# dominikh/jello

Hardware: AMD Instinct MI355X
Metric: Mpixels/sec fine-raster + paths/sec, 100k-path 4096^2 scene (higher is better)
Workload: dtype f32

## Files before the change

### jello_amd/csrc/kernels_coarse.hip

```cpp
#include <cstring>

#include "kcommon.h"

using namespace jk;
using namespace jd;

namespace {

struct Cmd {
    const JlConfig* cfg;
    JlBump* bump;
    Buf<uint32_t> ptcl;
    uint32_t cmd_offset, cmd_limit;
    uint32_t dyn_start;
    uint32_t chunk_base;
    uint32_t chunk_words;
    uint32_t seg_base, seg_used;
};

struct __attribute__((packed, aligned(4))) PtclQuad { uint32_t a, b, c, d; };
JD void ptcl_wr4(const Buf<uint32_t>& ptcl, uint32_t i, uint32_t a, uint32_t b, uint32_t c, uint32_t d) {
    if (i + 3u < ptcl.n && i + 3u >= i) {
        PtclQuad q; q.a = a; q.b = b; q.c = c; q.d = d;
        *(PtclQuad*)(ptcl.p + i) = q;
    } else {
        ptcl.wr(i, a); ptcl.wr(i + 1u, b); ptcl.wr(i + 2u, c); ptcl.wr(i + 3u, d);
    }
}

#ifndef COARSE_POOL_CHUNKS
#define COARSE_POOL_CHUNKS 16u
#endif
template <int MODE>
JD void alloc_cmd(Cmd& c, uint32_t size) {
    const bool need = c.cmd_offset + size >= c.cmd_limit;
    uint32_t new_cmd = c.dyn_start + c.chunk_base + c.chunk_words;
    if (MODE == 1) {
        if (need) {
            if (new_cmd + JL_PTCL_INCREMENT > c.cfg->ptcl_size) {
                new_cmd = 0u;
                atomicOr(&c.bump->failed, (uint32_t)JL_STAGE_COARSE);
            }
            c.ptcl.wr(c.cmd_offset, JL_CMD_JUMP);
            c.ptcl.wr(c.cmd_offset + 1u, new_cmd);
        }
    }
    c.chunk_words += need ? JL_PTCL_INCREMENT : 0u;
    c.cmd_offset = need ? new_cmd : c.cmd_offset;
    c.cmd_limit = need ? new_cmd + (JL_PTCL_INCREMENT - JL_PTCL_HEADROOM) : c.cmd_limit;
}

#define COARSE_UNROLL 4u
#ifndef COARSE_TILE_CACHE
#define COARSE_TILE_CACHE 1536u
#endif
#ifndef COARSE_WG_PER_CU
#define COARSE_WG_PER_CU 2u
#endif
#ifndef COARSE_MAX_SPLIT
#define COARSE_MAX_SPLIT 16u
#endif
#ifndef COARSE_PAR_WG_PER_CU
#define COARSE_PAR_WG_PER_CU 4u
#endif

#define CM_CLIP 1u
#define CM_BLEND 2u
#define CM_EVENODD_INCLUDE 4u
#define CM_EVENODD_FILL 8u
#define CM_PATH 16u
#define CM_BEGIN 32u
#define CM_END 64u
#define CM_NBRUSH_SHIFT 8u

#ifndef COARSE_TPL
#define COARSE_TPL 1u
#endif
#if COARSE_TPL != 1
#error "the write pass derives a tile's bases from its thread index: one tile per lane"
#endif
struct Walk {
    Cmd c;
    uint32_t blend_offset, clip_zero_depth, clip_depth, render_blend_depth, max_blend_depth;
    uint32_t tile_x, tile_y, my_xy, slot;
    bool has_tile;
    uint32_t slice_ix, bitmap, nz, el_next;
    uint4 q0, q2;
    JlTile tile;
};

struct CoarseReloc {
    uint32_t* arena_ctr;
    uint2* owner;
    unsigned long long* masks;
    uint32_t* aux;
    uint32_t* end_pos;
};

template <int MODE, bool CLIPS>
__global__ __launch_bounds__(JL_WG) void k_coarse(const JlConfig* __restrict__ cfg, Buf<uint32_t> scene, Buf<JlDrawMonoid> draw_monoids,
                                                  Buf<JlBinHeader> bin_headers, Buf<uint32_t> info_bin_data, Buf<JlPath> paths, Buf<JlTile> tiles,
                                                  JlBump* __restrict__ bump, Buf<uint32_t> ptcl, uint32_t* __restrict__ cnt_seg,
                                                  uint32_t* __restrict__ cnt_chunk, uint32_t* __restrict__ cnt_blend,
                                                  uint32_t* __restrict__ wg_tot, uint32_t n_wg, uint32_t bin_row0, uint32_t split, CoarseReloc R) {
    constexpr bool WRITE = MODE != 0;
    const uint32_t bin_y = blockIdx.y + bin_row0;
    const uint32_t part_rows = JL_N_TILE_Y / split, part_y0 = blockIdx.z * part_rows, part_y1 = part_y0 + part_rows;
    __shared__ uint32_t sh_bitmaps[8][JL_N_TILE];
    __shared__ uint32_t sh_part_count[JL_WG];
    __shared__ uint32_t sh_part_offsets[JL_WG];
    __shared__ uint32_t sh_drawobj_ix[JL_WG];
    __shared__ uint32_t sh_tile_count[JL_WG];
    __shared__ uint4 sh_r0[JL_WG];
    __shared__ uint4 sh_r1[JL_WG];
    __shared__ uint4 sh_r2[JL_WG];
    __shared__ uint32_t sh_scan[8];
    __shared__ uint32_t sh_red[12];
    constexpr bool PAR = MODE == 2;
    __shared__ uint2 sh_tile_cache[PAR ? 1u : COARSE_TILE_CACHE];
    __shared__ uint32_t sh_st[8][PAR ? JL_N_TILE : 1u];
    __shared__ uint8_t sh_list[JL_WG / 64][2][PAR ? JL_N_TILE : 1u];
    __shared__ uint32_t sh_pool[JL_WG / 64][2];
    if (PAR && threadIdx.x < JL_WG / 64) { sh_pool[threadIdx.x][0] = 0u; sh_pool[threadIdx.x][1] = 0u; }

    const uint32_t lid = threadIdx.x;
    const uint32_t width_in_bins = (cfg->width_in_tiles + JL_N_TILE_X - 1u) / JL_N_TILE_X;
    const uint32_t bin_ix = width_in_bins * bin_y + blockIdx.x;
    if (bin_ix * split + blockIdx.z >= n_wg) return;
    const uint32_t part_tiles = part_rows * JL_N_TILE_X, walkers = part_tiles / COARSE_TPL;
    Walk W[COARSE_TPL];
#pragma unroll
    for (uint32_t k = 0; k < COARSE_TPL; k++) {
        W[k].has_tile = lid < walkers;
        const uint32_t t = W[k].has_tile ? lid + k * walkers : 0u;
        W[k].tile_x = t % JL_N_TILE_X;
        W[k].tile_y = part_y0 + t / JL_N_TILE_X;
        W[k].my_xy = W[k].tile_y * JL_N_TILE_X + W[k].tile_x;
        W[k].slot = bin_ix * JL_N_TILE + W[k].my_xy;
    }

    {
        uint32_t failed = bump->failed & (JL_STAGE_BINNING | JL_STAGE_TILE_ALLOC | JL_STAGE_FLATTEN);
        if (bump->seg_counts > cfg->seg_counts_size) failed |= JL_STAGE_PATH_COUNT;
        if (failed != 0u) {
            if (WRITE) {
                if (blockIdx.x == 0u && blockIdx.y == 0u && lid == 0u) atomicOr(&bump->failed, failed);
            }
            if (MODE != 1) {
#pragma unroll
                for (uint32_t k = 0; k < COARSE_TPL; k++)
                    if (W[k].has_tile) { cnt_seg[W[k].slot] = 0u; cnt_chunk[W[k].slot] = 0u; cnt_blend[W[k].slot] = 0u; }
                if (lid < 3u) wg_tot[lid * n_wg + bin_ix * split + blockIdx.z] = 0u;
            }
            if (MODE == 2) {
#pragma unroll
                for (uint32_t k = 0; k < COARSE_TPL; k++)
                    if (W[k].has_tile) R.end_pos[W[k].slot] = 0xffffffffu;
            }
            return;
        }
    }
    const uint32_t n_partitions = (cfg->layout.n_drawobj + JL_N_TILE - 1u) / JL_N_TILE;
    const uint32_t bin_tile_x = JL_N_TILE_X * blockIdx.x;
    const uint32_t bin_tile_y = JL_N_TILE_Y * bin_y;
    const uint32_t BLEND_CLIP = (128u << 8) | 0u;
    uint32_t my_base_seg = 0u, my_base_chunk = 0u, my_base_blend = 0u;
    if (MODE == 1) {
        const uint32_t my_wg = bin_ix * split + blockIdx.z;
        MonoidK<3> before, all;
#pragma unroll
        for (int c = 0; c < 3; c++) { before.v[c] = 0u; all.v[c] = 0u; }
        const bool totals = blockIdx.x == 0u && blockIdx.y == 0u && blockIdx.z == 0u;
        for (uint32_t j = lid; j < (totals ? n_wg : my_wg); j += JL_WG) {
#pragma unroll
            for (int c = 0; c < 3; c++) {
                const uint32_t v = wg_tot[(uint32_t)c * n_wg + j];
                all.v[c] += v;
                if (j < my_wg) before.v[c] += v;
            }
        }
        const MonoidK<3> carry = block_reduce_monoid<3>(before, sh_red);
        __syncthreads();
        if (totals) {
            const MonoidK<3> t = block_reduce_monoid<3>(all, sh_red);
            if (lid == 0u) { bump->segments = t.v[0]; bump->ptcl = t.v[1]; bump->blend = t.v[2]; }
            __syncthreads();
        }
        const bool mine = W[0].has_tile;
        uint32_t tot;
        my_base_seg = carry.v[0] + block_excl_scan_u32(mine ? cnt_seg[W[0].slot] : 0u, sh_scan, &tot);
        __syncthreads();
        my_base_chunk = carry.v[1] + block_excl_scan_u32(mine ? cnt_chunk[W[0].slot] : 0u, sh_scan, &tot);
        __syncthreads();
        my_base_blend = carry.v[2] + block_excl_scan_u32(mine ? cnt_blend[W[0].slot] : 0u, sh_scan, &tot);
        __syncthreads();
    }
#pragma unroll
    for (uint32_t k = 0; k < COARSE_TPL; k++) {
        Walk& w = W[k];
        const uint32_t this_tile_ix = (bin_tile_y + w.tile_y) * cfg->width_in_tiles + bin_tile_x + w.tile_x;
        w.c.cfg = cfg; w.c.bump = bump; w.c.ptcl = ptcl;
        w.c.cmd_offset = this_tile_ix * JL_PTCL_INITIAL_ALLOC;
        w.c.cmd_limit = w.c.cmd_offset + (JL_PTCL_INITIAL_ALLOC - JL_PTCL_HEADROOM);
        w.c.dyn_start = cfg->width_in_tiles * cfg->height_in_tiles * JL_PTCL_INITIAL_ALLOC;
        w.c.chunk_base = my_base_chunk;
        w.c.chunk_words = 0u;
        w.c.seg_base = my_base_seg;
        w.c.seg_used = 0u;
        if (MODE == 2 && w.has_tile && bin_tile_x + w.tile_x < cfg->width_in_tiles && bin_tile_y + w.tile_y < cfg->height_in_tiles &&
            (size_t)this_tile_ix * JL_PTCL_INITIAL_ALLOC + JL_PTCL_INITIAL_ALLOC <= ptcl.n) {
            R.masks[(size_t)this_tile_ix * 2u] = 0ull;
            R.masks[(size_t)this_tile_ix * 2u + 1u] = 0ull;
        }
        w.clip_zero_depth = 0u; w.clip_depth = 0u; w.render_blend_depth = 0u; w.max_blend_depth = 0u;
        w.blend_offset = w.c.cmd_offset;
        w.c.cmd_offset += 1u;
        w.slice_ix = 7u; w.bitmap = 0u; w.nz = 0u; w.el_next = 0xffffffffu;
        w.q0 = make_uint4(0u, 0u, 0u, 0u); w.q2 = w.q0;
        w.tile.backdrop = 0; w.tile.segment_count_or_ix = 0u;
    }
    if constexpr (PAR) {
        if (W[0].has_tile) {
            sh_st[0][lid] = W[0].c.cmd_offset; sh_st[1][lid] = W[0].c.cmd_limit; sh_st[2][lid] = 0u; sh_st[3][lid] = 0u;
            sh_st[4][lid] = 0u; sh_st[5][lid] = 0u; sh_st[6][lid] = 0u; sh_st[7][lid] = 0u;
        }
    }
    uint32_t partition_ix = 0u, rd_ix = 0u, wr_ix = 0u, part_start_ix = 0u, ready_ix = 0u;

    auto gather = [&]() -> uint32_t {
        for (;;) {
            if (ready_ix == wr_ix && partition_ix < n_partitions) {
                part_start_ix = ready_ix;
                uint32_t count = 0u;
                if (partition_ix + lid < n_partitions) {
                    uint32_t in_ix = (partition_ix + lid) * JL_N_TILE + bin_ix;
                    JlBinHeader bh = bin_headers.rd(in_ix);
                    count = bh.element_count;
                    sh_part_offsets[lid] = bh.chunk_offset;
                }
                uint32_t tot;
                uint32_t excl = block_excl_scan_u32(count, sh_scan, &tot);
                sh_part_count[lid] = part_start_ix + excl + count;
                __syncthreads();
                ready_ix = sh_part_count[JL_WG - 1u];
                partition_ix += JL_WG;
            }
            uint32_t ix = rd_ix + lid;
            if (ix >= wr_ix && ix < ready_ix) {
                uint32_t part_ix = 0u;
                for (uint32_t i = 0; i < 8u; i++) {
                    uint32_t probe = part_ix + (128u >> i);
                    if (ix >= sh_part_count[probe - 1u]) part_ix = probe;
                }
                ix -= (part_ix > 0u) ? sh_part_count[part_ix - 1u] : part_start_ix;
                uint32_t offset = cfg->layout.bin_data_start + sh_part_offsets[part_ix];
                sh_drawobj_ix[lid] = info_bin_data.rd(offset + ix);
            }
            wr_ix = umin_(rd_ix + JL_N_TILE, ready_ix);
            if (wr_ix - rd_ix >= JL_N_TILE || (wr_ix >= ready_ix && partition_ix >= n_partitions)) break;
            __syncthreads();
        }
        return (lid + rd_ix < wr_ix) ? sh_drawobj_ix[lid] : 0xffffffffu;
    };
    uint32_t n_tag = JL_DRAWTAG_NOP;
    JlDrawMonoid n_dm;
    n_dm.path_ix = 0u; n_dm.clip_ix = 0u; n_dm.scene_offset = 0u; n_dm.info_offset = 0u;
    auto stage1 = [&](uint32_t obj) {
        n_tag = JL_DRAWTAG_NOP;
        if (obj != 0xffffffffu) {
            n_tag = scene.rd(cfg->layout.drawtag_base + obj);
            n_dm = draw_monoids.rd(obj);
        }
    };
    uint4 n_r0 = make_uint4(0u, 0u, 0u, 0u), n_r1 = make_uint4(0u, 0u, 0u, 0u), n_r2 = make_uint4(0u, 0u, 0u, 0u);
    uint32_t n_tile_count = 0u;
    auto stage2 = [&]() {
        const uint32_t tag = n_tag;
        n_tile_count = 0u;
        n_r0 = make_uint4(0u, 0u, 0u, 0u); n_r1 = make_uint4(0u, 0u, 0u, 0u); n_r2 = make_uint4(0u, 0u, 0u, 0u);
        if (tag != JL_DRAWTAG_NOP) {
            const JlDrawMonoid dm0 = n_dm;
            uint32_t path_ix = dm0.path_ix;
            uint32_t dd0 = cfg->layout.drawdata_base + dm0.scene_offset;
            const uint32_t di = dm0.info_offset;
            const uint32_t draw_flags = info_bin_data.rd(di);
            const uint4 sc = make_uint4(scene.rd(dd0), scene.rd(dd0 + 1u), scene.rd(dd0 + 2u), scene.rd(dd0 + 3u));
            uint32_t meta = (draw_flags & 1u) != 0u ? CM_EVENODD_INCLUDE : 0u;
            if ((tag & 1u) != 0u) {
                meta |= CM_CLIP;
                if (sc.x != BLEND_CLIP) meta |= CM_BLEND;
            }
            if (tag == JL_DRAWTAG_FILL_COLOR) {
                meta |= CM_PATH | (meta & CM_EVENODD_INCLUDE ? CM_EVENODD_FILL : 0u) | (5u << CM_NBRUSH_SHIFT);
                n_r0.y = JL_CMD_COLOR; n_r2 = sc;
            } else if (tag == JL_DRAWTAG_FILL_LIN_GRADIENT || tag == JL_DRAWTAG_FILL_RAD_GRADIENT || tag == JL_DRAWTAG_FILL_SWEEP_GRADIENT) {
                meta |= CM_PATH | (meta & CM_EVENODD_INCLUDE ? CM_EVENODD_FILL : 0u) | (3u << CM_NBRUSH_SHIFT);
                n_r0.y = tag == JL_DRAWTAG_FILL_LIN_GRADIENT ? JL_CMD_LIN_GRAD : (tag == JL_DRAWTAG_FILL_RAD_GRADIENT ? JL_CMD_RAD_GRAD : JL_CMD_SWEEP_GRAD);
                n_r2.x = sc.x; n_r2.y = di + 1u;
            } else if (tag == JL_DRAWTAG_FILL_IMAGE) {
                meta |= CM_PATH | (meta & CM_EVENODD_INCLUDE ? CM_EVENODD_FILL : 0u) | (2u << CM_NBRUSH_SHIFT);
                n_r0.y = JL_CMD_IMAGE; n_r2.x = di + 1u;
            } else if (CLIPS && tag == JL_DRAWTAG_BEGIN_CLIP) {
                meta |= CM_BEGIN | (1u << CM_NBRUSH_SHIFT);
                n_r0.y = JL_CMD_BEGIN_CLIP;
            } else if (CLIPS && tag == JL_DRAWTAG_END_CLIP) {
                meta |= CM_END | CM_PATH | (3u << CM_NBRUSH_SHIFT);
                n_r0.y = JL_CMD_END_CLIP; n_r2.x = sc.x; n_r2.y = sc.y;
            }
            n_r0.x = meta;
            JlPath path = paths.rd(path_ix);
            uint32_t stride = path.bbox[2] - path.bbox[0];
            n_r0.w = stride;
            int32_t dx = (int32_t)path.bbox[0] - (int32_t)bin_tile_x;
            int32_t dy = (int32_t)path.bbox[1] - (int32_t)bin_tile_y;
            int32_t x0 = iclamp_(dx, 0, JL_N_TILE_X);
            int32_t y0 = iclamp_(dy, (int32_t)part_y0, (int32_t)part_y1);
            int32_t x1 = iclamp_((int32_t)path.bbox[2] - (int32_t)bin_tile_x, 0, JL_N_TILE_X);
            int32_t y1 = iclamp_((int32_t)path.bbox[3] - (int32_t)bin_tile_y, (int32_t)part_y0, (int32_t)part_y1);
            {
                const uint32_t wdt = (uint32_t)(x1 - x0);
                n_r1.y = wdt | ((wdt ? (65536u + wdt - 1u) / wdt : 0u) << 5);
            }
            n_r1.x = (uint32_t)x0 | ((uint32_t)y0 << 16);
            n_tile_count = (uint32_t)(x1 - x0) * (uint32_t)(y1 - y0);
            n_r0.z = path.tiles - (uint32_t)(dy * (int32_t)stride + dx);
        }
    };
    stage1(gather());
    stage2();
    for (;;) {
        for (uint32_t i = 0; i < 8u; i++) sh_bitmaps[i][lid] = 0u;
        const uint32_t tile_count = n_tile_count;
        uint4 r0 = n_r0, r1 = n_r1, r2 = n_r2;
        uint32_t total_tile_count;
        uint32_t excl_tc = block_excl_scan_u32(tile_count, sh_scan, &total_tile_count);
        sh_tile_count[lid] = excl_tc + tile_count;
        r1.z = excl_tc;
        sh_r0[lid] = r0; sh_r1[lid] = r1; sh_r2[lid] = r2;
        __syncthreads();
        rd_ix += JL_N_TILE;
        const bool has_next = !(rd_ix >= ready_ix && partition_ix >= n_partitions);
        if (has_next) stage1(gather());
        uint32_t win_e0 = 0u, win_p0 = 0u;
        bool did_stage2 = false;
        for (;;) {
        uint32_t win_e1 = PAR ? JL_N_TILE : win_e0;
        for (uint32_t step = 256u; step > 0u && !PAR; step >>= 1)
            if (win_e1 + step <= JL_N_TILE && sh_tile_count[win_e1 + step - 1u] - win_p0 <= COARSE_TILE_CACHE) win_e1 += step;
        const uint32_t win_p1 = sh_tile_count[win_e1 - 1u];
        for (uint32_t base = win_p0; base < win_p1; base += COARSE_UNROLL * JL_N_TILE) {
            uint32_t p_el[COARSE_UNROLL], p_xy[COARSE_UNROLL], p_tile[COARSE_UNROLL];
            JlTile p_t[COARSE_UNROLL];
#pragma unroll
            for (uint32_t u = 0; u < COARSE_UNROLL; u++) {
                const uint32_t ix = base + u * JL_N_TILE + lid;
                p_el[u] = 0xffffffffu; p_xy[u] = 0u; p_tile[u] = 0u;
                p_t[u].backdrop = 0; p_t[u].segment_count_or_ix = 0u;
                if (ix < win_p1) {
                    uint32_t el_ix = 0u;
#pragma unroll
                    for (uint32_t i = 0; i < 8u; i++) {
                        uint32_t probe = el_ix + (128u >> i);
                        if (ix >= sh_tile_count[probe - 1u]) el_ix = probe;
                    }
                    const uint4 q0 = sh_r0[el_ix], q1 = sh_r1[el_ix];
                    uint32_t seq_ix = ix - q1.z;
                    uint32_t width = q1.y & 31u;
                    uint32_t row = (seq_ix * (q1.y >> 5)) >> 16;
                    uint32_t x = (q1.x & 0xffffu) + (seq_ix - row * width);
                    uint32_t y = (q1.x >> 16) + row;
                    p_el[u] = el_ix;
                    p_xy[u] = y * JL_N_TILE_X + x;
                    p_tile[u] = q0.z + q0.w * y + x;
                }
            }
#pragma unroll
            for (uint32_t u = 0; u < COARSE_UNROLL; u++)
                if (p_el[u] != 0xffffffffu) p_t[u] = tiles.rd(p_tile[u]);
#pragma unroll
            for (uint32_t u = 0; u < COARSE_UNROLL; u++) {
                if (p_el[u] == 0xffffffffu) continue;
                const uint32_t ix = base + u * JL_N_TILE + lid;
                const uint32_t el_ix = p_el[u];
                const JlTile tile = p_t[u];
                if (!PAR) sh_tile_cache[ix - win_p0] = make_uint2((uint32_t)tile.backdrop, tile.segment_count_or_ix);
                const uint32_t meta = sh_r0[el_ix].x;
                const bool is_clip = (meta & CM_CLIP) != 0u, is_blend = (meta & CM_BLEND) != 0u;
                const bool even_odd = (meta & CM_EVENODD_INCLUDE) != 0u;
                uint32_t n_segs = tile.segment_count_or_ix;
                int32_t bd = tile.backdrop;
                int32_t absbd = bd < 0 ? (int32_t)(0u - (uint32_t)bd) : bd;
                bool backdrop_clear = (even_odd ? (absbd & 1) : bd) == 0;
                bool include_tile = n_segs != 0u || (backdrop_clear == is_clip) || is_blend;
                if (include_tile) atomicOr(&sh_bitmaps[el_ix / 32u][p_xy[u]], 1u << (el_ix & 31u));
            }
        }
        if (has_next && !did_stage2) { stage2(); did_stage2 = true; }
        __syncthreads();
        if constexpr (PAR) {
            const uint32_t wv = lid >> 6, lane = lid & 63u;
            const uint64_t below = (1ull << lane) - 1ull, above = ~below & ~(1ull << lane);
            auto mbcnt64 = [&](uint64_t m) -> uint32_t { return __builtin_amdgcn_mbcnt_hi((uint32_t)(m >> 32), __builtin_amdgcn_mbcnt_lo((uint32_t)m, 0u)); };
            auto prepare = [&](uint32_t t, uint32_t buf, uint32_t& e_out, JlTile& tl) -> uint32_t {
                e_out = 0u; tl.backdrop = 0; tl.segment_count_or_ix = 0u;
                if (t >= part_tiles) return 0u;
                const uint32_t ty = part_y0 + t / JL_N_TILE_X, tx = t % JL_N_TILE_X, xy = ty * JL_N_TILE_X + tx;
                uint32_t n = 0u;
#pragma unroll
                for (uint32_t c = 0u; c < 4u; c++) {
                    const uint64_t m = (uint64_t)uni(sh_bitmaps[2u * c][xy]) | ((uint64_t)uni(sh_bitmaps[2u * c + 1u][xy]) << 32);
                    if (m != 0ull) {
                        if ((m >> lane) & 1ull) sh_list[wv][buf][(n + mbcnt64(m)) & 255u] = (uint8_t)(64u * c + lane);
                        n += (uint32_t)__builtin_popcountll(m);
                    }
                }
                wave_sync();
                if (lane < n) {
                    e_out = sh_list[wv][buf][lane];
                    const uint4 q0 = sh_r0[e_out];
                    tl = tiles.rd(q0.z + q0.w * ty + tx);
                }
                return n;
            };
            uint32_t nx_e; JlTile nx_tile;
            uint32_t nx_n = prepare(wv, 0u, nx_e, nx_tile);
            uint32_t buf = 0u;
            for (uint32_t t = wv; t < part_tiles; t += JL_WG / 64u, buf ^= 1u) {
                const uint32_t n = nx_n, e_first = nx_e;
                const JlTile tile_first = nx_tile;
                nx_n = prepare(t + JL_WG / 64u, buf ^ 1u, nx_e, nx_tile);
                if (n == 0u) continue;
                const uint32_t ty = part_y0 + t / JL_N_TILE_X, tx = t % JL_N_TILE_X;
                const uint32_t slot = bin_ix * JL_N_TILE + ty * JL_N_TILE_X + tx;
                uint32_t off = uni(sh_st[0][t]), lim = uni(sh_st[1][t]), chunkw = uni(sh_st[2][t]), segused = uni(sh_st[3][t]);
                uint32_t czd = uni(sh_st[4][t]), depth = uni(sh_st[5][t]), rbd = uni(sh_st[6][t]), maxbd = uni(sh_st[7][t]);
                const uint32_t dyn_start = cfg->width_in_tiles * cfg->height_in_tiles * JL_PTCL_INITIAL_ALLOC;
                for (uint32_t k0 = 0u; k0 < n; k0 += 64u) {
                    const bool live = k0 + lane < n;
                    uint32_t e = e_first;
                    JlTile tile = tile_first;
                    if (k0 != 0u) {
                        e = live ? sh_list[wv][buf][k0 + lane] : 0u;
                        tile.backdrop = 0; tile.segment_count_or_ix = 0u;
                        if (live) { const uint4 t0 = sh_r0[e]; tile = tiles.rd(t0.z + t0.w * ty + tx); }
                    }
                    const uint4 q0 = sh_r0[e], q2 = sh_r2[e];
                    const uint32_t meta = live ? q0.x : 0u;
                    const uint32_t n_segs = live ? tile.segment_count_or_ix : 0u;
                    const uint32_t is_begin = (meta / CM_BEGIN) & 1u, is_end = (meta / CM_END) & 1u, has_path = (meta / CM_PATH) & 1u;
                    const uint32_t has_segs = umin_(n_segs, 1u);
                    const uint32_t zero_tile = live ? 1u - umin_(n_segs | (uint32_t)tile.backdrop, 1u) : 0u;
                    const uint32_t dlt = is_begin - is_end;
                    const uint32_t d_incl = wave_incl_scan_u32(dlt);
                    const uint32_t D = depth + d_incl - dlt;
                    const uint64_t begins = __builtin_amdgcn_ballot_w64(is_begin != 0u);
                    const uint64_t zb = __builtin_amdgcn_ballot_w64((is_begin & zero_tile) != 0u);
                    uint32_t has_partner = 0u, partner_empty = 0u, matched = 0u;
                    for (uint64_t todo = begins; todo != 0ull;) {
                        const uint32_t L = (uint32_t)__builtin_amdgcn_readlane((int)D, (int)__builtin_ctzll(todo));
                        const bool bl_me = is_begin != 0u && D == L, el_me = is_end != 0u && D == L + 1u;
                        const uint64_t bl = __builtin_amdgcn_ballot_w64(bl_me), el = __builtin_amdgcn_ballot_w64(el_me);
                        if (el_me) {
                            const uint64_t c = bl & below;
                            if (c != 0ull) { has_partner = 1u; partner_empty = (uint32_t)(zb >> (63u - (uint32_t)__builtin_clzll(c))) & 1u; }
                        }
                        if (bl_me) {
                            const uint64_t ea = el & above, ba = bl & above;
                            matched = (ea != 0ull && (ba == 0ull || __builtin_ctzll(ea) < __builtin_ctzll(ba))) ? 1u : 0u;
                        }
                        todo &= ~bl;
                    }
                    const uint64_t ze = __builtin_amdgcn_ballot_w64((is_end & partner_empty) != 0u);
                    uint32_t skipped = mbcnt64(zb) > mbcnt64(ze) ? 1u : 0u;
                    uint32_t czd_out;
                    bool entered_persists = false;
                    if (czd != 0u) {
                        const uint64_t fin = __builtin_amdgcn_ballot_w64(is_end != 0u && has_partner == 0u && D == czd);
                        const uint32_t endl = fin != 0ull ? (uint32_t)__builtin_ctzll(fin) : 64u;
                        if (lane <= endl) skipped = 1u;
                        entered_persists = fin == 0ull;
                    }
                    if (entered_persists) {
                        czd_out = czd;
                    } else {
                        const uint64_t open_z = __builtin_amdgcn_ballot_w64((is_begin & zero_tile) != 0u && matched == 0u);
                        czd_out = open_z != 0ull ? (uint32_t)__builtin_amdgcn_readlane((int)D, (int)__builtin_ctzll(open_z)) + 1u : 0u;
                    }
                    const uint32_t active = 1u - skipped;
                    const uint32_t opened = is_begin & active & (1u - zero_tile), closes = is_end & active;
                    const uint32_t rd = opened - closes;
                    const uint32_t r_incl = wave_incl_scan_u32(rd);
                    const uint32_t peak = rbd + r_incl - rd + opened;
                    maxbd = umax_(maxbd, (uint32_t)__builtin_amdgcn_readlane((int)wave_incl_max_u32(peak), 63));
                    rbd += (uint32_t)__builtin_amdgcn_readlane((int)r_incl, 63);
                    depth += (uint32_t)__builtin_amdgcn_readlane((int)d_incl, 63);
                    czd = czd_out;
                    const uint32_t emit_path = active & has_path;
                    const uint32_t emit_brush = active & (1u - (is_begin & zero_tile));
                    const uint32_t s1 = emit_path * (1u + 3u * has_segs);
                    const uint32_t s2 = emit_brush * ((meta >> CM_NBRUSH_SHIFT) & 7u);
                    const uint32_t segs_here = emit_path * n_segs;
                    const uint32_t sg_incl = wave_incl_scan_u32(segs_here);
                    const uint32_t seg_ix = segused + sg_incl - segs_here;
                    segused += (uint32_t)__builtin_amdgcn_readlane((int)sg_incl, 63);
                    const uint32_t sz_incl = wave_incl_scan_u32(s1 + s2);
                    uint32_t o1 = off + sz_incl - (s1 + s2), o2 = o1 + s1;
                    uint32_t fl = 0u, fslot = 0u;
                    for (uint32_t guard = 0u; guard < 130u; guard++) {
                        const bool at1 = lane > fl || (lane == fl && fslot == 0u), at2 = lane >= fl;
                        const uint64_t m1 = __builtin_amdgcn_ballot_w64(s1 != 0u && at1 && o1 + s1 >= lim);
                        const uint64_t m2 = __builtin_amdgcn_ballot_w64(s2 != 0u && at2 && o2 + s2 >= lim);
                        if ((m1 | m2) == 0ull) break;
                        const uint32_t l1 = m1 != 0ull ? (uint32_t)__builtin_ctzll(m1) : 64u, l2 = m2 != 0ull ? (uint32_t)__builtin_ctzll(m2) : 64u;
                        const uint32_t bl = l1 <= l2 ? l1 : l2, bslot = l1 <= l2 ? 0u : 1u;
                        const uint32_t bo = (uint32_t)__builtin_amdgcn_readlane((int)(bslot == 0u ? o1 : o2), (int)bl);
                        uint32_t pn = uni(sh_pool[wv][0]), pe = uni(sh_pool[wv][1]);
                        if (pe - pn < JL_PTCL_INCREMENT) {
                            const uint32_t grab = COARSE_POOL_CHUNKS * JL_PTCL_INCREMENT;
                            uint32_t base = 0u;
                            if (lane == 0u) base = atomicAdd(R.arena_ctr, grab);
                            base = uni(base);
                            if (lane >= 1u && lane < COARSE_POOL_CHUNKS && dyn_start + base + lane * JL_PTCL_INCREMENT + JL_PTCL_INCREMENT <= ptcl.n)
                                R.owner[base / JL_PTCL_INCREMENT + lane] = make_uint2(0xffffffffu, 0u);
                            pn = base; pe = base + grab;
                        }
                        wave_sync();
                        if (lane == 0u) { sh_pool[wv][0] = pn + JL_PTCL_INCREMENT; sh_pool[wv][1] = pe; }
                        wave_sync();
                        uint32_t new_cmd = dyn_start + pn;
                        if (new_cmd + JL_PTCL_INCREMENT > ptcl.n || new_cmd + JL_PTCL_INCREMENT < new_cmd) {
                            new_cmd = 0u;
                        } else {
                            if (lane == 0u) R.owner[pn / JL_PTCL_INCREMENT] = make_uint2(slot, chunkw / JL_PTCL_INCREMENT);
                            if (lane < 4u) ((ulonglong2*)(R.masks + (size_t)(new_cmd >> 6) * 2u))[lane] = make_ulonglong2(0ull, 0ull);
                        }
                        if (lane == 0u) {
                            ptcl.wr(bo, JL_CMD_JUMP);
                            ptcl.wr(bo + 1u, new_cmd);
                            if (bo + 1u < ptcl.n) atomicOr(R.masks + (size_t)((bo + 1u) >> 6) * 2u + 1u, 1ull << ((bo + 1u) & 63u));
                        }
                        if (lane > bl || (lane == bl && bslot == 0u)) o1 = o1 - bo + new_cmd;
                        if (lane >= bl) o2 = o2 - bo + new_cmd;
                        lim = new_cmd + (JL_PTCL_INCREMENT - JL_PTCL_HEADROOM);
                        chunkw += JL_PTCL_INCREMENT;
                        fl = bl; fslot = bslot;
                    }
                    off = (uint32_t)__builtin_amdgcn_readlane((int)(o2 + s2), 63);
                    if (s1 == 4u) {
                        const uint32_t at = o1 + 2u;
                        if (at < ptcl.n) {
                            atomicOr(R.masks + (size_t)(at >> 6) * 2u, 1ull << (at & 63u));
                            R.aux[at >> 2] = q0.z + q0.w * ty + tx;
                        }
                        ptcl_wr4(ptcl, o1, JL_CMD_FILL, (n_segs << 1) | ((meta / CM_EVENODD_FILL) & 1u), seg_ix, (uint32_t)tile.backdrop);
                    } else if (s1 == 1u) {
                        ptcl.wr(o1, JL_CMD_SOLID);
                    }
                    if (s2 >= 4u) {
                        ptcl_wr4(ptcl, o2, q0.y, q2.x, q2.y, q2.z);
                        if (s2 == 5u) ptcl.wr(o2 + 4u, q2.w);
                    } else if (s2 != 0u) {
                        ptcl.wr(o2, q0.y);
                        if (s2 >= 2u) ptcl.wr(o2 + 1u, q2.x);
                        if (s2 >= 3u) ptcl.wr(o2 + 2u, q2.y);
                    }
                }
                if (lane == 0u) {
                    sh_st[0][t] = off; sh_st[1][t] = lim; sh_st[2][t] = chunkw; sh_st[3][t] = segused;
                    sh_st[4][t] = czd; sh_st[5][t] = depth; sh_st[6][t] = rbd; sh_st[7][t] = maxbd;
                }
            }
        } else {
        auto next_el = [&](Walk& w) -> uint32_t {
            if (w.bitmap == 0u) {
                if (w.nz == 0u) return 0xffffffffu;
                w.slice_ix = (uint32_t)__builtin_ctz(w.nz);
                w.nz &= w.nz - 1u;
                w.bitmap = sh_bitmaps[w.slice_ix][w.my_xy];
            }
            const uint32_t e = w.slice_ix * 32u + (uint32_t)__builtin_ctz(w.bitmap);
            w.bitmap &= w.bitmap - 1u;
            return e;
        };
        auto fetch = [&](Walk& w) {
            const uint32_t e = w.el_next & (JL_N_TILE - 1u);
            const uint4 q1 = sh_r1[e];
            w.q0 = sh_r0[e]; w.q2 = sh_r2[e];
            const uint32_t pair = q1.z + (w.tile_y - (q1.x >> 16)) * (q1.y & 31u) + (w.tile_x - (q1.x & 0xffffu));
            const uint2 tc = sh_tile_cache[umin_(pair - win_p0, COARSE_TILE_CACHE - 1u)];
            w.tile.backdrop = (int32_t)tc.x;
            w.tile.segment_count_or_ix = tc.y;
        };
        bool any = false;
#pragma unroll
        for (uint32_t k = 0; k < COARSE_TPL; k++) {
            Walk& w = W[k];
            const bool walks = w.has_tile && win_e0 < JL_N_TILE;
            w.slice_ix = walks ? win_e0 / 32u : 7u;
            uint32_t sl[8];
#pragma unroll
            for (uint32_t i = 0; i < 8u; i++) sl[i] = sh_bitmaps[i][w.my_xy];
            w.bitmap = 0u; w.nz = 0u;
#pragma unroll
            for (uint32_t i = 0; i < 8u; i++) {
                if (walks && i == w.slice_ix) w.bitmap = sl[i] & (0xffffffffu << (win_e0 & 31u));
                if (walks && i > w.slice_ix && sl[i] != 0u) w.nz |= 1u << i;
            }
            w.el_next = next_el(w);
            fetch(w);
            any = any || w.el_next != 0xffffffffu;
        }
        while (any) {
            any = false;
#pragma unroll
            for (uint32_t k = 0; k < COARSE_TPL; k++) {
                Walk& w = W[k];
                Cmd& c = w.c;
                const bool live = w.el_next != 0xffffffffu;
                const uint4 q0 = w.q0, q2 = w.q2;
                const JlTile tile = w.tile;
                if (live) w.el_next = next_el(w);
                fetch(w);
                any = any || w.el_next != 0xffffffffu;
                const uint32_t meta = live ? q0.x : 0u;
                const uint32_t n_segs = tile.segment_count_or_ix;
                const uint32_t is_begin = CLIPS ? (meta / CM_BEGIN) & 1u : 0u, is_end = CLIPS ? (meta / CM_END) & 1u : 0u;
                const uint32_t has_path = (meta / CM_PATH) & 1u;
                const uint32_t active = CLIPS ? 1u - umin_(w.clip_zero_depth, 1u) : 1u;
                const uint32_t has_segs = umin_(n_segs, 1u);
                const uint32_t zero_tile = 1u - umin_(n_segs | (uint32_t)tile.backdrop, 1u);
                if (CLIPS) {
                    const uint32_t open = is_begin & active;
                    const uint32_t opened = open & (1u - zero_tile);
                    const uint32_t ends_skip = is_end & (1u - active) & (1u - umin_(w.clip_depth ^ w.clip_zero_depth, 1u));
                    w.clip_zero_depth = (w.clip_zero_depth + (open & zero_tile) * (w.clip_depth + 1u)) * (1u - ends_skip);
                    w.render_blend_depth += opened;
                    w.max_blend_depth = umax_(w.max_blend_depth, w.render_blend_depth);
                    w.render_blend_depth -= is_end & active;
                    w.clip_depth += is_begin - is_end;
                }
                const uint32_t emit_path = active & has_path;
                const uint32_t emit_brush = active & (1u - (is_begin & zero_tile));
                const uint32_t s1 = emit_path * (1u + 3u * has_segs);
                const uint32_t seg_ix = c.seg_base + c.seg_used;
                c.seg_used += emit_path * n_segs;
                alloc_cmd<MODE>(c, s1);
                if (WRITE) {
                    const bool room = c.cmd_offset + 8u <= c.ptcl.n && c.cmd_offset + 8u > c.cmd_offset;
                    const uint32_t rule = (n_segs << 1) | ((meta / CM_EVENODD_FILL) & 1u);
                    if (s1 == 4u) {
                        const uint32_t tile_ix = q0.z + q0.w * w.tile_y + w.tile_x;
                        if (tiles.ok(tile_ix)) tiles.p[tile_ix].segment_count_or_ix = ~seg_ix;
                    }
                    if (s1 != 0u) {
                        PtclQuad q; q.a = has_segs ? JL_CMD_FILL : JL_CMD_SOLID; q.b = rule; q.c = seg_ix; q.d = (uint32_t)tile.backdrop;
                        if (room) *(PtclQuad*)(c.ptcl.p + c.cmd_offset) = q;
                        else if (s1 == 4u) ptcl_wr4(c.ptcl, c.cmd_offset, q.a, q.b, q.c, q.d);
                        else c.ptcl.wr(c.cmd_offset, q.a);
                    }
                }
                c.cmd_offset += s1;
                const uint32_t s2 = emit_brush * ((meta >> CM_NBRUSH_SHIFT) & 7u);
                alloc_cmd<MODE>(c, s2);
                if (WRITE) {
                    const bool room = c.cmd_offset + 8u <= c.ptcl.n && c.cmd_offset + 8u > c.cmd_offset;
                    if (s2 != 0u) {
                        if (room) {
                            PtclQuad q; q.a = q0.y; q.b = q2.x; q.c = q2.y; q.d = q2.z;
                            *(PtclQuad*)(c.ptcl.p + c.cmd_offset) = q;
                        } else {
                            c.ptcl.wr(c.cmd_offset, q0.y);
                            if (s2 >= 2u) c.ptcl.wr(c.cmd_offset + 1u, q2.x);
                            if (s2 >= 3u) c.ptcl.wr(c.cmd_offset + 2u, q2.y);
                            if (s2 >= 4u) c.ptcl.wr(c.cmd_offset + 3u, q2.z);
                        }
                    }
                    if (s2 == 5u) c.ptcl.wr(c.cmd_offset + 4u, q2.w);
                }
                c.cmd_offset += s2;
            }
        }
        }
        if (PAR || win_p1 >= total_tile_count) break;
        __syncthreads();
        win_e0 = win_e1; win_p0 = win_p1;
        }
        if (!has_next) break;
        __syncthreads();
    }
    if constexpr (PAR) {
        __syncthreads();
        if (W[0].has_tile) {
            W[0].c.cmd_offset = sh_st[0][lid]; W[0].c.chunk_words = sh_st[2][lid]; W[0].c.seg_used = sh_st[3][lid];
            W[0].max_blend_depth = sh_st[7][lid];
        }
    }
    MonoidK<3> my_tot;
    my_tot.v[0] = 0u; my_tot.v[1] = 0u; my_tot.v[2] = 0u;
#pragma unroll
    for (uint32_t k = 0; k < COARSE_TPL; k++) {
        Walk& w = W[k];
        if (!w.has_tile) continue;
        uint32_t scratch_size = 0u;
        const bool in_target = bin_tile_x + w.tile_x < cfg->width_in_tiles && bin_tile_y + w.tile_y < cfg->height_in_tiles;
        if (in_target && w.max_blend_depth > JL_BLEND_STACK_SPLIT) scratch_size = (w.max_blend_depth - JL_BLEND_STACK_SPLIT) * JL_TILE_WIDTH * JL_TILE_HEIGHT;
        if (MODE == 1) {
            if (in_target) {
                w.c.ptcl.wr(w.c.cmd_offset, JL_CMD_END);
                uint32_t blend_ix = 0u;
                if (scratch_size != 0u) {
                    blend_ix = my_base_blend;
                    if (blend_ix + scratch_size > cfg->blend_size) atomicOr(&bump->failed, (uint32_t)JL_STAGE_COARSE);
                }
                w.c.ptcl.wr(w.blend_offset, blend_ix);
            }
        } else {
            if (MODE == 2) {
                if (in_target) w.c.ptcl.wr(w.c.cmd_offset, JL_CMD_END);
                R.end_pos[w.slot] = in_target ? w.c.cmd_offset : 0xffffffffu;
            }
            cnt_seg[w.slot] = w.c.seg_used;
            cnt_chunk[w.slot] = w.c.chunk_words;
            cnt_blend[w.slot] = scratch_size;
            my_tot.v[0] = w.c.seg_used; my_tot.v[1] = w.c.chunk_words; my_tot.v[2] = scratch_size;
        }
    }
    if (MODE != 1) {
        const MonoidK<3> t = block_reduce_monoid<3>(my_tot, sh_red);
        if (lid < 3u) wg_tot[lid * n_wg + bin_ix * split + blockIdx.z] = lid == 0u ? t.v[0] : (lid == 1u ? t.v[1] : t.v[2]);
    }
}

__global__ __launch_bounds__(JL_WG) void k_coarse_bases(const JlConfig* __restrict__ cfg, JlBump* __restrict__ bump, const uint32_t* __restrict__ cnt_seg,
                                                        const uint32_t* __restrict__ cnt_chunk, const uint32_t* __restrict__ cnt_blend,
                                                        const uint32_t* __restrict__ wg_tot, uint32_t n_wg, uint32_t split, uint32_t* __restrict__ base_seg,
                                                        uint32_t* __restrict__ base_chunk, uint32_t* __restrict__ base_blend,
                                                        uint32_t* __restrict__ arena_ctr, uint32_t* __restrict__ arena_used, uint32_t arena_cap) {
    __shared__ uint32_t sh_scan[8];
    __shared__ uint32_t sh_red[12];
    const uint32_t lid = threadIdx.x, my_wg = blockIdx.x;
    const uint32_t bin_ix = my_wg / split, strip = my_wg % split;
    const uint32_t part_rows = JL_N_TILE_Y / split, part_tiles = part_rows * JL_N_TILE_X;
    MonoidK<3> before, all;
#pragma unroll
    for (int c = 0; c < 3; c++) { before.v[c] = 0u; all.v[c] = 0u; }
    const bool totals = my_wg == 0u;
    for (uint32_t j = lid; j < (totals ? n_wg : my_wg); j += JL_WG) {
#pragma unroll
        for (int c = 0; c < 3; c++) {
            const uint32_t v = wg_tot[(uint32_t)c * n_wg + j];
            all.v[c] += v;
            if (j < my_wg) before.v[c] += v;
        }
    }
    const MonoidK<3> carry = block_reduce_monoid<3>(before, sh_red);
    __syncthreads();
    if (totals) {
        const MonoidK<3> t = block_reduce_monoid<3>(all, sh_red);
        if (lid == 0u) {
            bump->segments = t.v[0]; bump->ptcl = t.v[1]; bump->blend = t.v[2];
            const uint64_t dyn_start = (uint64_t)cfg->width_in_tiles * cfg->height_in_tiles * JL_PTCL_INITIAL_ALLOC;
            if (t.v[1] != 0u && dyn_start + t.v[1] > cfg->ptcl_size) atomicOr(&bump->failed, (uint32_t)JL_STAGE_COARSE);
            *arena_used = *arena_ctr;
            if (*arena_ctr > arena_cap) {
                atomicOr(&bump->failed, (uint32_t)JL_STAGE_COARSE);
                bump->ptcl = umax_(bump->ptcl, *arena_ctr);
            }
        }
        __syncthreads();
    }
    const bool mine = lid < part_tiles;
    const uint32_t slot = bin_ix * JL_N_TILE + strip * part_tiles + lid;
    uint32_t tot;
    const uint32_t a = carry.v[0] + block_excl_scan_u32(mine ? cnt_seg[slot] : 0u, sh_scan, &tot);
    __syncthreads();
    const uint32_t b = carry.v[1] + block_excl_scan_u32(mine ? cnt_chunk[slot] : 0u, sh_scan, &tot);
    __syncthreads();
    const uint32_t d = carry.v[2] + block_excl_scan_u32(mine ? cnt_blend[slot] : 0u, sh_scan, &tot);
    if (mine) { base_seg[slot] = a; base_chunk[slot] = b; base_blend[slot] = d; }
}

__global__ __launch_bounds__(JL_WG) void k_coarse_relocate(const JlConfig* __restrict__ cfg, JlBump* __restrict__ bump, Buf<uint32_t> tmp, Buf<uint32_t> ptcl,
                                                           Buf<JlTile> tiles, const uint32_t* __restrict__ cnt_chunk, const uint32_t* __restrict__ cnt_blend,
                                                           const uint32_t* __restrict__ base_seg, const uint32_t* __restrict__ base_chunk,
                                                           const uint32_t* __restrict__ base_blend, const uint32_t* __restrict__ end_pos,
                                                           const uint2* __restrict__ owner, const unsigned long long* __restrict__ masks,
                                                           const uint32_t* __restrict__ aux, const uint32_t* __restrict__ arena_used,
                                                           uint32_t bin_row0, uint32_t bin_row1, uint32_t n_slots) {
    const uint32_t lane = lane_id();
    const uint32_t width_in_bins = (cfg->width_in_tiles + JL_N_TILE_X - 1u) / JL_N_TILE_X;
    const uint32_t dyn_start = cfg->width_in_tiles * cfg->height_in_tiles * JL_PTCL_INITIAL_ALLOC;
    const uint32_t slot0 = bin_row0 * width_in_bins * JL_N_TILE, slot1 = umin_(bin_row1 * width_in_bins * JL_N_TILE, n_slots);
    const uint32_t n_head_units = slot1 > slot0 ? (slot1 - slot0 + 3u) / 4u : 0u;
    const uint32_t n_chunks = umin_(*arena_used, tmp.n > dyn_start ? tmp.n - dyn_start : 0u) / JL_PTCL_INCREMENT;
    const uint32_t units = n_head_units + n_chunks;
    const uint32_t n_waves = (gridDim.x * JL_WG) >> 6;
    const uint32_t part = lane >> 4, wl = (lane & 15u) * 4u;
    for (uint32_t u = (blockIdx.x * JL_WG + threadIdx.x) >> 6; u < units; u += n_waves) {
        uint32_t slot, src, dst, next_chunk;
        bool head = u < n_head_units, live = true;
        if (head) {
            slot = slot0 + u * 4u + part;
            live = slot < slot1;
            const uint32_t bin_ix = slot / JL_N_TILE, xy = slot % JL_N_TILE;
            const uint32_t tx = (bin_ix % width_in_bins) * JL_N_TILE_X + xy % JL_N_TILE_X, ty = (bin_ix / width_in_bins) * JL_N_TILE_Y + xy / JL_N_TILE_X;
            live = live && tx < cfg->width_in_tiles && ty < cfg->height_in_tiles;
            if (live) live = end_pos[slot] != 0xffffffffu;
            src = dst = (ty * cfg->width_in_tiles + tx) * JL_PTCL_INITIAL_ALLOC + wl;
            next_chunk = 0u;
        } else {
            const uint32_t c = u - n_head_units;
            const uint2 ow = owner[c];
            slot = ow.x;
            src = dyn_start + c * JL_PTCL_INCREMENT + part * 64u + wl;
            dst = 0u; next_chunk = 0u;
            live = slot >= slot0 && slot < slot1;
            if (live) {
                const uint32_t k = ow.y, n_k = cnt_chunk[slot] / JL_PTCL_INCREMENT;
                live = k < n_k && !(k + 1u == n_k && (src & ~63u) > end_pos[slot]);
                dst = dyn_start + base_chunk[slot] + k * JL_PTCL_INCREMENT + part * 64u + wl;
                next_chunk = k + 1u;
            }
        }
        const bool in_range = src + 3u < tmp.n, fetch = live && in_range;
        const unsigned long long raw_jm = fetch ? masks[(size_t)(src >> 6) * 2u + 1u] : 0ull;
        const unsigned long long raw_fm = fetch ? masks[(size_t)(src >> 6) * 2u] : 0ull;
        const uint4 in = fetch ? *(const uint4*)(tmp.p + src) : make_uint4(0u, 0u, 0u, 0u);
        const uint32_t end_at = fetch ? end_pos[slot] : 0u;
        bool dead_block = false;
        if (!head) {
            const uint32_t lo = (uint32_t)raw_jm, hi = (uint32_t)(raw_jm >> 32);
            const bool j0 = ((uint32_t)__builtin_amdgcn_readlane((int)lo, 0) | (uint32_t)__builtin_amdgcn_readlane((int)hi, 0)) != 0u;
            const bool j1 = ((uint32_t)__builtin_amdgcn_readlane((int)lo, 16) | (uint32_t)__builtin_amdgcn_readlane((int)hi, 16)) != 0u;
            const bool j2 = ((uint32_t)__builtin_amdgcn_readlane((int)lo, 32) | (uint32_t)__builtin_amdgcn_readlane((int)hi, 32)) != 0u;
            dead_block = (part > 0u && j0) || (part > 1u && j1) || (part > 2u && j2);
        }
        if (!fetch || dead_block) continue;
        const bool ends_here = head ? (end_at >> 6) == (src >> 6) : (end_at >= (src & ~63u) - part * 64u && end_at - ((src & ~63u) - part * 64u) < JL_PTCL_INCREMENT);
        bool keep[4];
#pragma unroll
        for (uint32_t e = 0; e < 4u; e++) {
            const uint32_t ix = (src & 63u) + e;
            keep[e] = (raw_jm & ((1ull << ix) - 1ull)) == 0ull && !(ends_here && src + e > end_at);
        }
        if (!(keep[0] || keep[1] || keep[2] || keep[3])) continue;
        const unsigned long long fm = raw_fm >> (src & 63u), jm = raw_jm >> (src & 63u);
        uint32_t w[4] = {in.x, in.y, in.z, in.w};
        if (((fm | jm) & 15ull) != 0ull || (head && wl == 0u)) {
// ... 111 lines not shown
```

Before: 20980.

## Count coarse PTCL chunk usage with bitplane popcounts instead of per-element walk

Adds a packed counting path for the no-clip count pass of the coarse kernel. Each tile records include and has-segment bits in 64-bit shared bitmaps, and per-element command sizes are built from ballot bitplanes. The chunk allocation is then computed with popcounts and a binary search for the crossing points, instead of walking every element per tile. Segment totals are gathered with shared atomics. This drops the tile cache windowing and the per-element fetch loop, but adds 64-bit shared atomics and assumes the command-size model exactly matches what the write pass emits.

```diff
diff --git a/jello_amd/csrc/coarse_pack.h b/jello_amd/csrc/coarse_pack.h
--- /dev/null
+++ b/jello_amd/csrc/coarse_pack.h
@@ -0,0 +1,75 @@
+#pragma once
+#include <stdint.h>
+
+#ifndef CP_INLINE
+#define CP_INLINE static inline
+#endif
+
+namespace cpack {
+
+enum { CP_CHUNK = 256, CP_HEADROOM = 2, CP_HEAD = 64 };
+#define CP_R_HEAD (CP_HEAD - 1 - CP_HEADROOM)
+#define CP_R_CHUNK (CP_CHUNK - CP_HEADROOM)
+
+struct State {
+    uint32_t r, chunk_words;
+};
+
+CP_INLINE State cp_start() {
+    State s;
+    s.r = CP_R_HEAD; s.chunk_words = 0u;
+    return s;
+}
+
+CP_INLINE void cp_cmd(State& s, uint32_t size) {
+    const bool need = size >= s.r;
+    s.chunk_words += need ? (uint32_t)CP_CHUNK : 0u;
+    s.r = (need ? (uint32_t)CP_R_CHUNK : s.r) - size;
+}
+
+struct Word {
+    uint32_t p1, p3, q1, q2, q4;
+};
+CP_INLINE Word cp_word(uint32_t inc, uint32_t seg, uint32_t has_path, uint32_t nb0, uint32_t nb1, uint32_t nb2) {
+    Word w;
+    w.p1 = inc & has_path; w.p3 = inc & seg & has_path; w.q1 = inc & nb0; w.q2 = inc & nb1; w.q4 = inc & nb2;
+    return w;
+}
+CP_INLINE uint32_t cp_words(const Word& w, uint32_t m) {
+    return (uint32_t)__builtin_popcount(w.p1 & m) + 3u * (uint32_t)__builtin_popcount(w.p3 & m) + (uint32_t)__builtin_popcount(w.q1 & m) +
+           2u * (uint32_t)__builtin_popcount(w.q2 & m) + 4u * (uint32_t)__builtin_popcount(w.q4 & m);
+}
+
+CP_INLINE void cp_advance(State& s, const uint32_t* inc, const uint32_t* seg, uint32_t stride, const uint32_t* has_path, const uint32_t* nb0,
+                          const uint32_t* nb1, const uint32_t* nb2) {
+    uint32_t t[8], total = 0u;
+#pragma unroll
+    for (uint32_t i = 0; i < 8u; i++) {
+        t[i] = cp_words(cp_word(inc[i * stride], seg[i * stride], has_path[i], nb0[i], nb1[i], nb2[i]), 0xffffffffu);
+        total += t[i];
+    }
+    uint32_t placed = 0u;
+    while (total - placed >= s.r) {
+        const uint32_t target = placed + s.r;
+        uint32_t wi = 0u, below = 0u, acc = 0u;
+#pragma unroll
+        for (uint32_t i = 0; i < 7u; i++) {
+            acc += t[i];
+            if (acc < target) { wi = i + 1u; below = acc; }
+        }
+        const Word w = cp_word(inc[wi * stride], seg[wi * stride], has_path[wi], nb0[wi], nb1[wi], nb2[wi]);
+        uint32_t b = 0u;
+#pragma unroll
+        for (uint32_t step = 16u; step != 0u; step >>= 1)
+            if (below + cp_words(w, (1u << (b + step)) - 1u) < target) b += step;
+        const uint32_t before = below + cp_words(w, (1u << b) - 1u);
+        s.r -= before - placed;
+        const uint32_t s1 = ((w.p1 >> b) & 1u) + 3u * ((w.p3 >> b) & 1u), s2 = ((w.q1 >> b) & 1u) + 2u * ((w.q2 >> b) & 1u) + 4u * ((w.q4 >> b) & 1u);
+        cp_cmd(s, s1);
+        cp_cmd(s, s2);
+        placed = before + s1 + s2;
+    }
+    s.r -= total - placed;
+}
+
+}
diff --git a/jello_amd/csrc/kernels_coarse.hip b/jello_amd/csrc/kernels_coarse.hip
--- a/jello_amd/csrc/kernels_coarse.hip
+++ b/jello_amd/csrc/kernels_coarse.hip
@@ -1,6 +1,8 @@
 #include <cstring>
 
 #include "kcommon.h"
+#define CP_INLINE JD
+#include "coarse_pack.h"
 
 using namespace jk;
 using namespace jd;
@@ -62,6 +64,10 @@
 #endif
 #ifndef COARSE_PAR_WG_PER_CU
 #define COARSE_PAR_WG_PER_CU 4u
+#endif
+
+#ifndef COARSE_COUNT_PACK
+#define COARSE_COUNT_PACK 1
 #endif
 
 #define CM_CLIP 1u
@@ -104,20 +110,26 @@
                                                   uint32_t* __restrict__ cnt_chunk, uint32_t* __restrict__ cnt_blend,
                                                   uint32_t* __restrict__ wg_tot, uint32_t n_wg, uint32_t bin_row0, uint32_t split, CoarseReloc R) {
     constexpr bool WRITE = MODE != 0;
+    constexpr bool PACK = MODE == 0 && !CLIPS && COARSE_COUNT_PACK != 0;
     const uint32_t bin_y = blockIdx.y + bin_row0;
     const uint32_t part_rows = JL_N_TILE_Y / split, part_y0 = blockIdx.z * part_rows, part_y1 = part_y0 + part_rows;
-    __shared__ uint32_t sh_bitmaps[8][JL_N_TILE];
+    __shared__ uint32_t sh_bitmaps[8][PACK ? 1u : JL_N_TILE];
     __shared__ uint32_t sh_part_count[JL_WG];
     __shared__ uint32_t sh_part_offsets[JL_WG];
     __shared__ uint32_t sh_drawobj_ix[JL_WG];
     __shared__ uint32_t sh_tile_count[JL_WG];
     __shared__ uint4 sh_r0[JL_WG];
     __shared__ uint4 sh_r1[JL_WG];
-    __shared__ uint4 sh_r2[JL_WG];
+    __shared__ uint4 sh_r2[PACK ? 1u : JL_WG];
     __shared__ uint32_t sh_scan[8];
     __shared__ uint32_t sh_red[12];
     constexpr bool PAR = MODE == 2;
-    __shared__ uint2 sh_tile_cache[PAR ? 1u : COARSE_TILE_CACHE];
+    constexpr bool NOWIN = PAR || PACK;
+    __shared__ uint2 sh_tile_cache[NOWIN ? 1u : COARSE_TILE_CACHE];
+    __shared__ unsigned long long sh_bits[8][PACK ? JL_N_TILE : 1u];
+    __shared__ uint32_t sh_segsum[PACK ? JL_N_TILE : 1u];
+    __shared__ uint32_t sh_plane[4][8];
+    if (PACK) sh_segsum[threadIdx.x] = 0u;
     __shared__ uint32_t sh_st[8][PAR ? JL_N_TILE : 1u];
     __shared__ uint8_t sh_list[JL_WG / 64][2][PAR ? JL_N_TILE : 1u];
     __shared__ uint32_t sh_pool[JL_WG / 64][2];
@@ -225,6 +237,7 @@
             sh_st[4][lid] = 0u; sh_st[5][lid] = 0u; sh_st[6][lid] = 0u; sh_st[7][lid] = 0u;
         }
     }
+    cpack::State pack_st = cpack::cp_start();
     uint32_t partition_ix = 0u, rd_ix = 0u, wr_ix = 0u, part_start_ix = 0u, ready_ix = 0u;
 
     auto gather = [&]() -> uint32_t {
@@ -284,7 +297,7 @@
             uint32_t dd0 = cfg->layout.drawdata_base + dm0.scene_offset;
             const uint32_t di = dm0.info_offset;
             const uint32_t draw_flags = info_bin_data.rd(di);
-            const uint4 sc = make_uint4(scene.rd(dd0), scene.rd(dd0 + 1u), scene.rd(dd0 + 2u), scene.rd(dd0 + 3u));
+            const uint4 sc = PACK ? make_uint4(0u, 0u, 0u, 0u) : make_uint4(scene.rd(dd0), scene.rd(dd0 + 1u), scene.rd(dd0 + 2u), scene.rd(dd0 + 3u));
             uint32_t meta = (draw_flags & 1u) != 0u ? CM_EVENODD_INCLUDE : 0u;
             if ((tag & 1u) != 0u) {
                 meta |= CM_CLIP;
@@ -329,14 +342,32 @@
     stage1(gather());
     stage2();
     for (;;) {
-        for (uint32_t i = 0; i < 8u; i++) sh_bitmaps[i][lid] = 0u;
+        if (PACK) {
+            for (uint32_t i = 0; i < 8u; i++) sh_bits[i][lid] = 0ull;
+        } else {
+            for (uint32_t i = 0; i < 8u; i++) sh_bitmaps[i][lid] = 0u;
+        }
         const uint32_t tile_count = n_tile_count;
         uint4 r0 = n_r0, r1 = n_r1, r2 = n_r2;
         uint32_t total_tile_count;
         uint32_t excl_tc = block_excl_scan_u32(tile_count, sh_scan, &total_tile_count);
         sh_tile_count[lid] = excl_tc + tile_count;
         r1.z = excl_tc;
-        sh_r0[lid] = r0; sh_r1[lid] = r1; sh_r2[lid] = r2;
+        sh_r0[lid] = r0; sh_r1[lid] = r1;
+        if (PACK) {
+            const uint32_t nbrush = (r0.x >> CM_NBRUSH_SHIFT) & 7u;
+            const uint64_t b[4] = {__builtin_amdgcn_ballot_w64((r0.x & CM_PATH) != 0u), __builtin_amdgcn_ballot_w64((nbrush & 1u) != 0u),
+                                   __builtin_amdgcn_ballot_w64((nbrush & 2u) != 0u), __builtin_amdgcn_ballot_w64((nbrush & 4u) != 0u)};
+            if ((lid & 63u) == 0u) {
+#pragma unroll
+                for (uint32_t p = 0; p < 4u; p++) {
+                    sh_plane[p][(lid >> 6) * 2u] = (uint32_t)b[p];
+                    sh_plane[p][(lid >> 6) * 2u + 1u] = (uint32_t)(b[p] >> 32);
+                }
+            }
+        } else {
+            sh_r2[lid] = r2;
+        }
         __syncthreads();
         rd_ix += JL_N_TILE;
         const bool has_next = !(rd_ix >= ready_ix && partition_ix >= n_partitions);
@@ -344,8 +375,8 @@
         uint32_t win_e0 = 0u, win_p0 = 0u;
         bool did_stage2 = false;
         for (;;) {
-        uint32_t win_e1 = PAR ? JL_N_TILE : win_e0;
-        for (uint32_t step = 256u; step > 0u && !PAR; step >>= 1)
+        uint32_t win_e1 = NOWIN ? JL_N_TILE : win_e0;
+        for (uint32_t step = 256u; step > 0u && !NOWIN; step >>= 1)
             if (win_e1 + step <= JL_N_TILE && sh_tile_count[win_e1 + step - 1u] - win_p0 <= COARSE_TILE_CACHE) win_e1 += step;
         const uint32_t win_p1 = sh_tile_count[win_e1 - 1u];
         for (uint32_t base = win_p0; base < win_p1; base += COARSE_UNROLL * JL_N_TILE) {
@@ -383,7 +414,7 @@
                 const uint32_t ix = base + u * JL_N_TILE + lid;
                 const uint32_t el_ix = p_el[u];
                 const JlTile tile = p_t[u];
-                if (!PAR) sh_tile_cache[ix - win_p0] = make_uint2((uint32_t)tile.backdrop, tile.segment_count_or_ix);
+                if (!NOWIN) sh_tile_cache[ix - win_p0] = make_uint2((uint32_t)tile.backdrop, tile.segment_count_or_ix);
                 const uint32_t meta = sh_r0[el_ix].x;
                 const bool is_clip = (meta & CM_CLIP) != 0u, is_blend = (meta & CM_BLEND) != 0u;
                 const bool even_odd = (meta & CM_EVENODD_INCLUDE) != 0u;
@@ -392,7 +423,12 @@
                 int32_t absbd = bd < 0 ? (int32_t)(0u - (uint32_t)bd) : bd;
                 bool backdrop_clear = (even_odd ? (absbd & 1) : bd) == 0;
                 bool include_tile = n_segs != 0u || (backdrop_clear == is_clip) || is_blend;
-                if (include_tile) atomicOr(&sh_bitmaps[el_ix / 32u][p_xy[u]], 1u << (el_ix & 31u));
+                if (PACK) {
+                    if (include_tile) atomicOr(&sh_bits[el_ix / 32u][p_xy[u]], (1ull | (n_segs != 0u ? 1ull << 32 : 0ull)) << (el_ix & 31u));
+                    if (n_segs != 0u && (meta & CM_PATH) != 0u) atomicAdd(&sh_segsum[p_xy[u]], n_segs);
+                } else {
+                    if (include_tile) atomicOr(&sh_bitmaps[el_ix / 32u][p_xy[u]], 1u << (el_ix & 31u));
+                }
             }
         }
         if (has_next && !did_stage2) { stage2(); did_stage2 = true; }
@@ -570,6 +606,11 @@
                     sh_st[4][t] = czd; sh_st[5][t] = depth; sh_st[6][t] = rbd; sh_st[7][t] = maxbd;
                 }
             }
+        } else if constexpr (PACK) {
+            if (W[0].has_tile) {
+                const uint32_t* bits = (const uint32_t*)&sh_bits[0][W[0].my_xy];
+                cpack::cp_advance(pack_st, bits, bits + 1, 2u * JL_N_TILE, sh_plane[0], sh_plane[1], sh_plane[2], sh_plane[3]);
+            }
         } else {
         auto next_el = [&](Walk& w) -> uint32_t {
             if (w.bitmap == 0u) {
@@ -681,7 +722,7 @@
             }
         }
         }
-        if (PAR || win_p1 >= total_tile_count) break;
+        if (NOWIN || win_p1 >= total_tile_count) break;
         __syncthreads();
         win_e0 = win_e1; win_p0 = win_p1;
         }
@@ -694,6 +735,9 @@
             W[0].c.cmd_offset = sh_st[0][lid]; W[0].c.chunk_words = sh_st[2][lid]; W[0].c.seg_used = sh_st[3][lid];
             W[0].max_blend_depth = sh_st[7][lid];
         }
+    }
+    if constexpr (PACK) {
+        if (W[0].has_tile) { W[0].c.chunk_words = pack_st.chunk_words; W[0].c.seg_used = sh_segsum[W[0].my_xy]; }
     }
     MonoidK<3> my_tot;
     my_tot.v[0] = 0u; my_tot.v[1] = 0u; my_tot.v[2] = 0u;
```

After: 21190, median of 6. About the same (+1.0%).
